# ttanv/funsearch-kubernetes-simulator

Hardware: AMD Instinct MI355X
Metric: policy evals/sec on 8,152-pod Alibaba trace at 1/2/4/8 GPUs; champion util/frag (higher is better)
Workload: dtype fp64; 1 GPU; model=composite_linear policy family, exact replay (reference-bit-identical scores), global_batch=49152, seq_len=8152, parallelism=islands: 4/GPU x 1 rank(s), single rank (no collectives), dist_backend=none, world_size=1, candidates_per_island=12288, backend=hip, heap_mode=auto, islands_async=True

## Files before the change

### csrc/hip/engine_host.hip.h

```cpp
#pragma once

#include <hip/hip_runtime.h>
#include <pybind11/numpy.h>
#include <rocprofiler-sdk-roctx/roctx.h>
#include <pybind11/pybind11.h>

#include <algorithm>
#include <cmath>
#include <cstdio>
#include <cstdlib>
#include <mutex>
#include <cstring>
#include <memory>
#include <string>
#include <vector>

namespace fks_host {

namespace py = pybind11;
using namespace fksd;

#define HIP_OK(expr)                                                                    \
  do {                                                                                  \
    hipError_t _e = (expr);                                                             \
// ... 704 lines not shown
      if (c5) {
        if (s.fam_spec != FAM_COMPOSITE_LINEAR || !g)
          throw std::invalid_argument("256-node profiling: composite batch with verified reciprocals and an HBM heap");
        HIP_OK(fksk::launch_c5_prof(P, lds, s.stream, a));
      } else {
        HIP_OK(fksk::launch_builtin_prof(g, P, lds, s.stream, a));
      }
    }
    finish(s);
    py::array_t<uint64_t> prof({(py::ssize_t)P, (py::ssize_t)8});
    HIP_OK(hipMemcpyAsync(prof.mutable_data(), s.prof.p, (size_t)P * 64, hipMemcpyDeviceToHost, s.stream));
    py::array_t<double> tab = wait(0);
    HIP_OK(hipStreamSynchronize(s.stream));
    return py::make_tuple(tab, prof);
  }

  py::tuple profile_rows(py::array_t<int32_t, py::array::c_style | py::array::forcecast> fam,
                         py::array_t<double, py::array::c_style | py::array::forcecast> weights) {
    if (!rows_ok_) throw std::invalid_argument("row kernel needs <= 16 nodes");
    HIP_OK(hipSetDevice(device_));
    Slot& s = idle_slot(0);
    stage_builtin(s, fam.data(), weights.data(), (int)fam.size());
    const int waves = launch_rows(s, true);
    finish(s);
    py::array_t<uint64_t> prof({(py::ssize_t)waves, (py::ssize_t)kRowProfWords});
    HIP_OK(hipMemcpyAsync(prof.mutable_data(), s.prof.p, (size_t)waves * 8 * kRowProfWords, hipMemcpyDeviceToHost,
                          s.stream));
    py::array_t<double> tab = wait(0);
    HIP_OK(hipStreamSynchronize(s.stream));
    return py::make_tuple(tab, prof);
  }

  py::dict info() const {
    py::dict d;
    d["device"] = device_; d["arch"] = arch_; d["num_cus"] = num_cus_;
    d["heap_bytes_per_policy"] = (int64_t)heap_bytes_;
    d["lds_heap_ok"] = lds_heap_ok_;
    d["npass"] = npass_;
    d["heap_mode"] = heap_mode_;
    d["n_slots"] = (int)slots_.size();
    d["heap_top_hbm"] = heap_top_for(0, false);
    d["row_kernel_ok"] = rows_ok_;
    d["row_kernel"] = row_mode_;
    d["row_heap_top"] = row_top();
    d["row_waves_per_cu"] = row_layout(FAM_COMPOSITE_LINEAR).second;
    d["row_wave_share"] = row_share_;
    d["fast_div"] = (int)W_.fast_div;
    d["cap_recips"] = W_.cap_recip[1] != 0.0;
    d["frag_recip"] = W_.z_tg != 0.0;
    d["row_composite_waves"] = comp_waves_;
    d["stack_bytes"] = (int64_t)stack_bytes_;
    d["row_flat"] = row_flat_;
    d["native_rows_last"] = last_native_rows_;
    d["native_waves_last"] = last_native_waves_;
    d["native_duo_top_last"] = last_duo_top_;
    d["native_duo_per_cu_last"] = last_duo_per_cu_;
    d["native_duo_reg_cap"] = fksk::native_duo_blocks_per_cu(0);
    d["native_inflight"] = native_inflight_;
    d["max_events"] = (int64_t)max_events_;
    d["wave_duo"] = wave_duo_;
    d["wave_duo_heap_top"] = npass_ >= 4 ? heap_top_for(0, false, true) : 0;
    size_t mfree = 0, mtotal = 0;
    if (hipMemGetInfo(&mfree, &mtotal) == hipSuccess) {
      d["mem_used_mb"] = (int64_t)((mtotal - mfree) >> 20);
      d["mem_total_mb"] = (int64_t)(mtotal >> 20);
    }
    return d;
  }

  bool would_use_hbm(int P) const { return use_gheap(P); }
  bool would_use_rows(int) const { return use_rows(); }
  int n_slots() const { return (int)slots_.size(); }

 private:
  static constexpr size_t kMaxLds = 160 * 1024;
  static constexpr int kWeightWords = kWeights;
  static constexpr size_t kSimds = 4;
  static constexpr size_t kPoliciesPerCu = kSimds * FKS_LIGHT_WAVES;
  static constexpr size_t kNp2PoliciesPerCu = kSimds * FKS_NP2_WAVES;
  static constexpr size_t kNp4PoliciesPerCu = kSimds * FKS_NP4_WAVES;
  static constexpr size_t kNp4DuoPoliciesPerCu = 2 * FKS_NP4_DUO_WAVES;
  static constexpr size_t kVmPoliciesPerCu = kSimds * FKS_VM_WAVES;

  void prepare_recips(py::dict d) {
    auto i32 = [&](const char* k) {
      return py::array_t<int32_t, py::array::c_style | py::array::forcecast>(d[k].cast<py::array>());
    };
    const auto ct = i32("cpu_total"), cl = i32("cpu_left"), mt = i32("mem_total"), ml = i32("mem_left"), ng = i32("ngpus");
    const auto pod = i32("pod");
    const int nn = (int)ct.size(), np = W_.n_pods;
    std::vector<std::pair<std::pair<int64_t, int64_t>, double>> cache;
    bool ok = true;
    std::vector<double> rec((size_t)nn * 3, 0.0), cm((size_t)std::max(np, 1), 0.0);
    std::vector<int32_t> per_class(256, 0);
    for (int r = 0; r < np; ++r) {
      const int32_t c = pod.data()[4 * r], m = pod.data()[4 * r + 1];
      ok = ok && c >= 0 && m >= 0;
      cm[r] = (double)c / (double)(m > 1 ? m : 1);
      const uint32_t pw = (uint32_t)pod.data()[4 * r + 3];
      if ((pw >> 16) & 0xFF) ++per_class[pw >> 24];
    }
    max_class_pods_ = *std::max_element(per_class.begin(), per_class.end());
    {
      const auto gl = i32("gpu_left"), gt = i32("gml_total"), gml = i32("gml_left");
      bool b = ok;
      for (int n = 0; n < nn && b; ++n) {
// ... 246 lines not shown
    if (profiled) HIP_OK(fksk::launch_builtin_rows_prof(kf, P, waves, s.queue.as<uint32_t>(), s.qbase, lds, s.stream, a));
    else HIP_OK(fksk::launch_builtin_rows(kf, P, waves, s.queue.as<uint32_t>(), s.qbase, lds, s.stream, a));
    s.qbase += (uint32_t)P + (uint32_t)waves * kRowsPerWave;
    return waves;
  }

  int duo_top(int want) const {
    const int entries = row_heap_entries(W_.n_pods);
    if (native_duo_top_ >= 0) {
      int T = 1;
      while (T < entries - 1 && 2 * T + 1 <= native_duo_top_) T = 2 * T + 1;
      return T;
    }
    const int reg_cap = std::max(1, fksk::native_duo_blocks_per_cu(0));
    const int need = std::min(reg_cap, std::max(1, (want + num_cus_ - 1) / std::max(1, num_cus_)));
    auto per_cu = [&](int T) {
      const size_t lds = duo_lds_bytes(W_.n_pods, T);
      if (lds > kMaxLds) return 0;
      return std::max(0, fksk::native_duo_blocks_per_cu(lds));
    };
    int T = 63;
    while (T < entries - 1 && per_cu(2 * T + 1) >= std::max(2, need)) T = 2 * T + 1;
    return T;
  }

  void launch_rows_native(Slot& s, int P, size_t fn_bytes, const int64_t* kc_dev, bool profiled = false) {
    const int ra = native_rows_opt_ > 0 ? native_rows_opt_ : (native_duo_ || P <= 2 * num_cus_ ? 1 : kRowsPerWave);
    DevWorkload Wl = W_;
    const int entries = row_heap_entries(W_.n_pods);
    if (ra == 1 && native_duo_) {
      const int T = duo_top(std::max(P, native_inflight_));
      Wl.heap_top = T;
      last_duo_top_ = T;
      last_duo_per_cu_ = fksk::native_duo_blocks_per_cu(duo_lds_bytes(W_.n_pods, T));
      const size_t lds = duo_lds_bytes(W_.n_pods, T);
      if (lds > kMaxLds) throw std::invalid_argument("native duo layout exceeds the 160 KiB LDS");
      s.gheap.reserve((size_t)entries * 8 * (size_t)P);
      if (profiled) s.prof.reserve((size_t)P * 128);
      const fksk::BuiltinArgs a{Wl, nullptr, nullptr, nullptr, nullptr, s.res.as<DevResult>(),
                                s.gheap.as<uint64_t>(), profiled ? s.prof.as<uint64_t>() : nullptr,
                                s.h_tab.dev<double>()};
      s.fused_table = true;
      const RowNativeArgs nat{s.h_in.dev<const uint64_t>(), kc_dev,
                              reinterpret_cast<const int32_t*>(s.h_in.dev<char>() + fn_bytes), nullptr, max_events_};
      if (std::getenv("FKS_DEBUG_LAUNCH"))
        std::fprintf(stderr, "[fks] native duo: P=%d T=%d lds=%zu per_cu=%d stream=%p\n", P, T, lds,
                     last_duo_per_cu_, (void*)s.stream);
      HIP_OK(fksk::launch_native_duo(P, lds, s.stream, a, nat));
      last_native_rows_ = 0;
      last_native_waves_ = 2 * P;
      return;
    }
    int T = 1;
    while (T < entries - 1 && rows_lds_bytes(W_.n_pods, 2 * T + 1, ra, true) <= kMaxLds / 2) T = 2 * T + 1;
    Wl.heap_top = T;
    const size_t lds = rows_lds_bytes(W_.n_pods, T, ra, true) + (profiled ? kRowProfBytes : 0);
    if (lds > kMaxLds) throw std::invalid_argument("native row kernel layout exceeds the 160 KiB LDS");
    const int per_cu = std::max(1, std::min(fksk::native_rows_waves_per_cu(lds), (int)(kMaxLds / ((lds + 2047) & ~size_t(2047)))));
    const int cap = std::max(1, (int)(row_share_ * per_cu * num_cus_));
    const int waves = std::max(1, std::min((P + ra - 1) / ra, cap));
    s.gheap.reserve((size_t)entries * 8 * (size_t)waves * kRowsPerWave);
    if (profiled) s.prof.reserve((size_t)waves * 8 * kRowProfWords);
    const fksk::BuiltinArgs a{Wl, nullptr, nullptr, nullptr, nullptr, s.res.as<DevResult>(),
                              s.gheap.as<uint64_t>(), profiled ? s.prof.as<uint64_t>() : nullptr, s.h_tab.dev<double>()};
    s.fused_table = true;
    const RowNativeArgs nat{s.h_in.dev<const uint64_t>(), kc_dev,
                            reinterpret_cast<const int32_t*>(s.h_in.dev<char>() + fn_bytes)};
    if (std::getenv("FKS_DEBUG_LAUNCH"))
      std::fprintf(stderr, "[fks] native rows: P=%d rows=%d waves=%d T=%d lds=%zu qbase=%u stream=%p\n", P, ra, waves, T,
                   lds, s.qbase, (void*)s.stream);
    HIP_OK(fksk::launch_native_rows(P, waves, ra, s.queue.as<uint32_t>(), s.qbase, lds, s.stream, a, nat));
    s.qbase += (uint32_t)P + (uint32_t)waves * (uint32_t)ra;
    last_native_rows_ = ra;
    last_native_waves_ = waves;
  }

  void launch_vm(Slot& s, int nregs) {
    const int P = s.P;
    const bool g = use_gheap(P);
    const DevWorkload Wl = launch_workload(g, nregs, true);
    const size_t lds = lds_bytes(g, Wl.heap_top, nregs);
    if (lds > kMaxLds) throw std::invalid_argument("heap + VM registers exceed the 160 KiB LDS");
    uint64_t* gh = g ? gheap_for(s, P) : nullptr;
    const fksk::VmArgs a{Wl, nullptr, table(s), s.res.as<DevResult>(), budget_, nregs, gh, nullptr};
    HIP_OK(fksk::launch_vm(npass_, g, P, lds, s.stream, a));
  }

  static void zero_queue(Slot& s) {
    static const uint64_t zeros[8] = {0, 0, 0, 0, 0, 0, 0, 0};
    HIP_OK(hipMemcpyAsync(s.queue.p, zeros, 64, hipMemcpyHostToDevice, s.stream));
    HIP_OK(hipStreamSynchronize(s.stream));
  }

  void finish(Slot& s) {
    const int P = s.P;
    if (!s.fused_table)
      hipLaunchKernelGGL(k_eval_reduce, dim3((P + 63) / 64), dim3(64), 0, s.stream, s.res.as<DevResult>(),
                         s.h_tab.dev<double>(), P);
    s.fused_table = false;
    HIP_OK(hipGetLastError());
    HIP_OK(hipEventRecord(s.done, s.stream));
    s.busy = true;
  }

  int device_ = 0;
  std::vector<std::unique_ptr<Slot>> slots_;
  DevWorkload W_;
  int npass_ = 1;
  size_t heap_bytes_ = 0, delmap_bytes_ = 0;
  bool lds_heap_ok_ = true;
  bool rows_ok_ = false;
  bool state_bounded_ = false;
  std::string row_mode_ = "auto";
  int row_top_opt_ = -1;
  double row_share_ = 1.0;
  bool native_duo_ = true;
  int native_rows_opt_ = 0;
  int native_inflight_ = 0;
  int native_duo_top_ = -1;
  int last_duo_top_ = 0, last_duo_per_cu_ = 0;
  int last_native_rows_ = 0, last_native_waves_ = 0;
  size_t row_min_lds_ = 0;
  int32_t max_class_pods_ = 0;
  int32_t max_gpu_milli_ = 0;
  static constexpr size_t kJitStackBytes = 2048;
  size_t stack_bytes_ = 0;
  bool row_flat_ = true;
  int comp_waves_ = 5;
  mutable std::vector<std::pair<int, int>> row_layout_cache_ = std::vector<std::pair<int, int>>(8, {0, 0});
  int num_cus_ = 0;
  std::string arch_;
  std::string heap_mode_ = "auto";
  int64_t budget_ = 0;
  uint32_t max_events_ = 0;
  int heap_top_opt_ = -1;
  bool partial_delmap_off_ = false;
  bool wave_duo_ = false;
  std::vector<void*> owned_;
};

}
```

### csrc/hip/replay_duo.hip.h

```cpp
#pragma once

#include "replay_rows.hip.h"

namespace fksd {

constexpr int kDuoRing = 64;
#ifndef FKS_DUO_SLEEP
#define FKS_DUO_SLEEP 1
#endif
constexpr uint32_t kDuoSpinCap = 1u << 26;
enum DuoReply : int32_t { DUO_NONE = 0, DUO_PLACED = 1, DUO_FAIL = 2, DUO_ABORT = 3 };

struct DuoBox {
  uint64_t ev[kDuoRing];
  uint64_t item;
  uint32_t head;
  uint32_t tail;
  uint32_t rseq;
  int32_t code;
  uint32_t term;
  uint32_t sabort;
  int32_t h_exc, n_repush, n_dropped;
};
constexpr int kDuoNodeInts = 16;
constexpr size_t kDuoSBytes = (size_t)kRow * kDuoNodeInts * 4 + (size_t)kRow * 32;
__host__ __device__ inline size_t duo_lds_bytes(int n_pods, int T) {
  return rows_lds_bytes(n_pods, T, 1, true) + ((sizeof(DuoBox) + 15) & ~size_t(15)) + kDuoSBytes;
}

__device__ __forceinline__ uint32_t duo_ld(FKS_LDS uint32_t* p) {
  return __hip_atomic_load(p, __ATOMIC_ACQUIRE, __HIP_MEMORY_SCOPE_WORKGROUP);
}
__device__ __forceinline__ void duo_st(FKS_LDS uint32_t* p, uint32_t v) {
  __hip_atomic_store(p, v, __ATOMIC_RELEASE, __HIP_MEMORY_SCOPE_WORKGROUP);
}


__device__ __forceinline__ void duo_reset(FKS_LDS DuoBox* box) {
  box->item = 0; box->head = 0; box->tail = 0; box->rseq = 0; box->code = DUO_NONE; box->term = 0;
  box->sabort = 0;
  box->h_exc = EXC_NONE; box->n_repush = 0; box->n_dropped = 0;
}

__device__ __forceinline__ bool duo_publish(FKS_LDS DuoBox* box, bool first, uint32_t k, uint32_t& tail_seen,
                                            uint64_t key, int32_t& hexc) {
  uint32_t spins = 0;
  while (k - tail_seen >= (uint32_t)kDuoRing) {
    tail_seen = duo_ld(&box->tail);
    if (k - tail_seen < (uint32_t)kDuoRing) break;
    if (duo_ld(&box->sabort)) return false;
    __builtin_amdgcn_s_sleep(FKS_DUO_SLEEP);
    if (++spins > kDuoSpinCap) { hexc = EXC_TIMEOUT; return false; }
  }
  if (first) box->ev[k % kDuoRing] = key;
  if (first) duo_st(&box->head, k + 1);
  return true;
}

__device__ __forceinline__ bool duo_verdict(FKS_LDS DuoBox* box, uint32_t k, int32_t& hexc) {
  uint32_t spins = 0;
  while (duo_ld(&box->rseq) != k + 1) {
    if (duo_ld(&box->sabort)) { hexc = EXC_TIMEOUT; return false; }
    __builtin_amdgcn_s_sleep(FKS_DUO_SLEEP);
    if (++spins > kDuoSpinCap) { hexc = EXC_TIMEOUT; return false; }
  }
  return true;
}

__device__ __forceinline__ void duo_term(FKS_LDS DuoBox* box, int32_t hexc, int n_repush, int n_dropped) {
  box->h_exc = hexc;
  box->n_repush = n_repush;
  box->n_dropped = n_dropped;
  duo_st(&box->term, 1u);
}

__device__ __forceinline__ bool duo_next(FKS_LDS DuoBox* box, uint32_t k, int32_t& exc) {
  uint32_t spins = 0;
  for (;;) {
    if (duo_ld(&box->head) > k) return true;
    if (duo_ld(&box->term)) return duo_ld(&box->head) > k;
// ... 69 lines not shown
    }
    pos = next;
    if (taken < 6) break;
  }
  if (target < 0) target = pos;
  if (j == 0) { hp.st(target, last); hp.mark(target, last); }
}

template <bool PROF = false>
__device__ void replay_duo(const DevWorkload& W, const DevWorkload* Wdev, uint64_t* gheap, DevResult* out,
                           RowNativeArgs nat, double* table, uint64_t* prof_out = nullptr, int slot = -1,
                           int hslot = -1) {
  uint64_t pacc[8] = {0, 0, 0, 0, 0, 0, 0, 0};
  uint64_t plast = 0;
  auto mark = [&](int ph) {
    if constexpr (PROF) {
      const uint64_t now = __builtin_amdgcn_s_memtime();
      pacc[ph] += now - plast;
      plast = now;
    }
  };
  auto flush = [&](int wv) {
    if constexpr (PROF) {
      if (lane_id() < 8) {
        uint64_t v = 0;
#pragma unroll
        for (int i = 0; i < 8; ++i) v = lane_id() == i ? pacc[i] : v;
        prof_out[16 * (size_t)blockIdx.x + 8 * wv + lane_id()] = v;
      }
    }
  };
  auto cold = [&]() {
    const DevWorkload* g = reinterpret_cast<const DevWorkload*>(uniu64(reinterpret_cast<uint64_t>(Wdev)));
    asm volatile("" : "+s"(g));
    return const_ptr(g);
  };
  extern __shared__ uint64_t lds_raw[];
  const int lane = lane_id();
  const int wave = (int)(threadIdx.x >> 6);
  const int p = slot >= 0 ? slot : (int)blockIdx.x;
  const int hs = hslot >= 0 ? hslot : p;
  const int N = W.n_pods;
  const int T = W.heap_top;
  const int lb = W.low_bits, nb = W.node_bits, rb = W.rank_bits;
  const int tshift = rb + lb;
  const uint64_t time_max = (W.time_bits >= 63) ? ~0ull : ((1ull << W.time_bits) - 1);
  int jv = lane & 15;
  const bool node_valid = jv < W.n_nodes;

  FKS_LDS uint64_t* lds = lds_ptr(lds_raw);
  FKS_LDS int32_t* cls_lds = reinterpret_cast<FKS_LDS int32_t*>(lds + kRowsPerWave * kWeights);
  FKS_LDS char* rowbase = reinterpret_cast<FKS_LDS char*>(lds + kRowsPerWave * kWeights) + kRowClassBytes;
  FKS_LDS int32_t* ntab = cls_lds + kRow * kRowClassSlots;
  FKS_LDS int64_t* kcp = reinterpret_cast<FKS_LDS int64_t*>(rowbase + rows_row_bytes(N, T));
  FKS_LDS DuoBox* box = reinterpret_cast<FKS_LDS DuoBox*>(reinterpret_cast<FKS_LDS char*>(lds) + rows_lds_bytes(N, T, 1, true));
  FKS_LDS int32_t* sstate = reinterpret_cast<FKS_LDS int32_t*>(reinterpret_cast<FKS_LDS char*>(box) +
                                                                ((sizeof(DuoBox) + 15) & ~size_t(15)));
  FKS_LDS uint64_t* sacc = reinterpret_cast<FKS_LDS uint64_t*>(sstate + kRow * kDuoNodeInts);

  if (wave == 0) {
    if (lane < W.n_classes) cls_lds[lane] = *global_ptr(&W.class_value[lane]);
    fill_node_tables(W, ntab, lane);
    if (lane == 0) {
      box->item = 0; box->head = 0; box->tail = 0; box->rseq = 0; box->code = DUO_NONE; box->term = 0;
      box->sabort = 0;
      box->h_exc = EXC_NONE; box->n_repush = 0; box->n_dropped = 0;
    }
  } else {
    const FKS_GLOBAL int64_t* ksrc = global_ptr(nat.kc + *global_ptr(&nat.koff[p]));
    for (int i = lane; i < kKcLds; i += kWave) kcp[i] = ksrc[i];
  }
  __syncthreads();
  if (wave == 1 && lane >= kRow) return;

  if (wave == 0) {
    RowHeap heap;
    heap.delmap = reinterpret_cast<FKS_LDS uint32_t*>(rowbase);
    heap.top = reinterpret_cast<FKS_LDS uint64_t*>(rowbase + (size_t)lds_delmap_words(N) * 4);
    heap.h = global_ptr(gheap + (size_t)hs * row_heap_entries(N));
    heap.bind();
    heap.T = T;
    heap.lb = lb;
    heap.j = jv;
    heap.rbase = 0;
    heap.anc = heap.dir = 0;
    uint64_t anc64 = 0, dir64 = 0;
    for (int x = lane; x > 0 && x < 63; x = (x - 1) >> 1) {
      const int a = (x - 1) >> 1;
      anc64 |= 1ull << a;
      if ((x & 1) == 0) dir64 |= 1ull << a;
    }
    const FKS_GLOBAL u64x2* heap_src = reinterpret_cast<const FKS_GLOBAL u64x2*>(global_ptr(W.heap0p));
    for (int i = lane; i < row_heap_entries(N) / 2; i += kWave) {
      const u64x2 v = heap_src[i];
      if (2 * i < T + 1) *reinterpret_cast<FKS_LDS u64x2*>(heap.top + 2 * i) = v;
      else *reinterpret_cast<FKS_GLOBAL u64x2*>(heap.h + 2 * i) = v;
    }
    for (int i = lane; i < lds_delmap_words(N); i += kWave) heap.delmap[i] = 0u;
    __builtin_amdgcn_s_waitcnt(0);
    int n = N, n_repush = 0, n_dropped = 0;
    int32_t hexc = EXC_NONE;
    uint32_t k = 0, tail_seen = 0;
    auto publish = [&](uint64_t key) -> bool {
      uint32_t spins = 0;
      while (k - tail_seen >= (uint32_t)kDuoRing) {
        tail_seen = duo_ld(&box->tail);
        if (k - tail_seen < (uint32_t)kDuoRing) break;
        if (duo_ld(&box->sabort)) return false;
// ... 386 lines not shown
```

### csrc/hip/replay_rows.hip.h

```cpp
#pragma once

#include "replay.hip.h"
#include "scorers.hip.h"
#include "jit_abi.h"

namespace fksd {

#ifndef FKS_ROW_FLAT
#define FKS_ROW_FLAT 1
#endif
constexpr int kFamNative = 100;
constexpr int kRowCompositeW5 = 5;
constexpr int kRowCompositeSplit = 6;
struct RowNativeArgs {
  const uint64_t* fn;
  const int64_t* kc;
  const int32_t* koff;
  const uint32_t* abort = nullptr;
  uint32_t max_events = 0;
};
struct ServiceCtl {
  uint32_t* claimed;
  const uint32_t* published;
  const uint32_t* stop;
  uint32_t* done;
  const uint32_t* qslot;
  uint32_t* started;
  uint32_t nq;
  uint32_t max_idle_polls;
  uint64_t* cost;
};

constexpr int kRow = 16;
constexpr int kRowsPerWave = 4;
constexpr int kRowClassSlots = 4;
constexpr int kRowMaxHeap = (1 << 17) - 2;

__host__ __device__ inline int row_heap_entries(int n_pods) { return (n_pods + 2 + 63) & ~63; }

__device__ __forceinline__ uint32_t row_ballot(bool p, int rbase) {
  return (uint32_t)(ballot(p) >> rbase) & 0xFFFFu;
}
template <int N>
__device__ __forceinline__ uint32_t row_ror32(uint32_t v) {
  return (uint32_t)__builtin_amdgcn_mov_dpp((int)v, 0x120 + N, 0xF, 0xF, false);
}
template <int N>
__device__ __forceinline__ uint64_t row_ror64(uint64_t v) {
  return ((uint64_t)row_ror32<N>((uint32_t)(v >> 32)) << 32) | row_ror32<N>((uint32_t)v);
}
__device__ __forceinline__ uint64_t row_max_u64(uint64_t v) {
  uint64_t o;
  o = row_ror64<8>(v); v = o > v ? o : v;
  o = row_ror64<4>(v); v = o > v ? o : v;
  o = row_ror64<2>(v); v = o > v ? o : v;
  o = row_ror64<1>(v); v = o > v ? o : v;
  return v;
}
__device__ __forceinline__ int64_t row_sum_i64(int64_t v) {
  uint64_t u = (uint64_t)v;
  u += row_ror64<8>(u);
  u += row_ror64<4>(u);
  u += row_ror64<2>(u);
  u += row_ror64<1>(u);
  return (int64_t)u;
}
__device__ __forceinline__ int row_read(int v, int rbase, int k) {
  return __builtin_amdgcn_ds_bpermute((rbase + k) << 2, v);
}

typedef uint64_t u64x2 __attribute__((ext_vector_type(2)));

template <bool FLAT = FKS_ROW_FLAT != 0>
struct RowHeapT {
  FKS_GLOBAL uint64_t* h;
  FKS_LDS uint64_t* top;
  int T;
  FKS_LDS uint32_t* delmap;
  int lb;
  int j, rbase;
  uint32_t anc, dir;

  uint64_t* gtop;
  uint64_t* gh;
  __device__ __forceinline__ void bind() {
    gtop = (uint64_t*)top;
    gh = (uint64_t*)h;
  }
  __device__ __forceinline__ uint64_t* slot(int i) const { return (i < T ? gtop : gh) + (i + 1); }
  __device__ __forceinline__ uint64_t ld(int i) const {
    if constexpr (FLAT) return *slot(i);
    else return i < T ? top[i + 1] : h[i + 1];
  }
  __device__ __forceinline__ void st(int i, uint64_t v) const {
    if constexpr (FLAT) {
      *slot(i) = v;
    } else {
      if (i < T) top[i + 1] = v;
      else h[i + 1] = v;
    }
  }
  __device__ __forceinline__ u64x2 ld_pair(int c) const {
    if constexpr (FLAT) return *reinterpret_cast<const u64x2*>(slot(c));
    if (c < T) return *reinterpret_cast<const FKS_LDS u64x2*>(top + c + 1);
    return *reinterpret_cast<const FKS_GLOBAL u64x2*>(h + c + 1);
  }
  __device__ __forceinline__ void mark(int pos, uint64_t v) const {
    const uint32_t bit = 1u << (pos & 31);
    const uint32_t data = (v & 3) == kDelKind ? bit : 0u;
    const uint32_t addr = (uint32_t)(uintptr_t)(delmap + (pos >> 5));
    asm volatile("ds_mskor_b32 %0, %1, %2" ::"v"(addr), "v"(bit), "v"(data) : "memory");
  }

  __device__ void pop_reinsert(int n, uint64_t last) const {
    const int k = j == 0 ? 0 : j < 3 ? 1 : j < 7 ? 2 : 3;
    const int ki = j - ((1 << k) - 1);
    constexpr int kRounds = 5;
    int pos = 0, target = -1;
#pragma unroll
    for (int rd = 0; rd < kRounds; ++rd) {
      if (2 * pos + 1 >= n) break;
      const int q = ((pos + 1) << k) - 1 + ki;
      const int c = 2 * q + 1;
      const bool valid = j < 15 && c < n;
      uint64_t vl = ~0ull, vr = ~0ull;
      if (valid) {
        const u64x2 pr = ld_pair(c);
        vl = pr.x;
        vr = pr.y;
      }
      const bool go_r = valid && (c + 1 < n) && !(vl < vr);
      const uint32_t m = row_ballot(go_r, rbase);
      const bool on = valid && ((m ^ dir) & anc) == 0;
      const uint32_t onm = row_ballot(on, rbase);
      const uint64_t v = go_r ? vr : vl;
      const uint32_t g = row_ballot(on && last < v, rbase);
      const int jl = g ? __ffs(g) - 1 : kRow;
      if (on && j < jl) {
        st(q, v);
        mark(q, v);
      }
      if (g) {
        target = row_read(q, rbase, jl);
        break;
      }
      const int jd = 31 - __clz(onm);
      const int nk = row_read(((c + (int)go_r) << 2) | k, rbase, jd);
      pos = nk >> 2;
      if ((nk & 3) < 3) break;
    }
    if (target < 0) target = pos;
    if (j == 0) { st(target, last); mark(target, last); }
  }

  __device__ void push(int n, uint64_t item) const {
    const int l = j + 1;
    const int anc = ((n + 1) >> l) - 1;
    const bool valid = n > 0 && anc >= 0;
    const uint64_t v = valid ? ld(anc) : 0;
    const bool gt = valid && item < v;
    const int J = __popc(row_ballot(gt, rbase));
    const int dst = ((n + 1) >> (l - 1)) - 1;
    if (gt) { st(dst, v); mark(dst, v); }
    const int aJ = J == 0 ? n : ((n + 1) >> J) - 1;
    if (j == 0) { st(aJ, item); mark(aJ, item); }
  }

  __device__ int first_deletion(int n) const {
    const int words = (n + 31) >> 5;
    for (int base = 0; base < words; base += kRow) {
      const int wi = base + j;
      uint32_t w = wi < words ? delmap[wi] : 0u;
      if (wi == words - 1 && (n & 31)) w &= (1u << (n & 31)) - 1;
      const uint32_t b = row_ballot(w != 0, rbase);
      if (b) {
        const int fl = __ffs(b) - 1;
        const uint32_t fw = (uint32_t)row_read((int)w, rbase, fl);
        return ((base + fl) << 5) + (__ffs(fw) - 1);
      }
    }
    return -1;
  }
};
using RowHeap = RowHeapT<>;

struct RowAcc {
  uint64_t lo, hi;
  int32_t count;
  int32_t inexact;
  __device__ void init() { lo = hi = 0; count = 0; inexact = 0; }
  __device__ void add(int k, double v, int j) {
    const bool mine = j == k;
    const uint64_t bits = (uint64_t)__double_as_longlong(v);
    if (mine) ++count;
    if (bits == 0) return;
    const int E = (int)(bits >> 52);
    const uint64_t M = (bits & ((1ull << 52) - 1)) | (1ull << 52);
    const int shift = E - 979;
    bool bad = E == 0 || E >= 0x7FF || shift > 126 - 53;
    uint64_t tl, th;
    if (shift >= 0) {
      tl = shift < 64 ? M << shift : 0ull;
      th = shift == 0 ? 0ull : shift < 64 ? M >> (64 - shift) : M << (shift - 64);
    } else {
      bad = bad || shift <= -53 || (M & ((1ull << (-shift)) - 1)) != 0;
      tl = M >> (-shift & 63);
      th = 0;
    }
    if (bad) {
      if (mine) inexact |= 1;
      return;
    }
    if (mine) {
      lo += tl;
      hi += th + (lo < tl);
      if (hi >> 62) inexact |= 1;
    }
  }
  __device__ void add_unit(int k, double v, int j) {
    const bool mine = j == k;
    const uint64_t bits = (uint64_t)__double_as_longlong(v);
    if (mine) ++count;
    if (bits == 0) return;
    const int s = (int)(bits >> 52) - 979;
    const uint64_t M = (bits & ((1ull << 52) - 1)) | (1ull << 52);
    const uint64_t tl = M << (s & 63), th = M >> ((64 - s) & 63);
    if (mine) {
      if (s < 13 || s > 44) inexact |= 1;
      lo += tl;
      hi += th + (lo < tl);
    }
// ... 28 lines not shown
constexpr int kNodeRecips = 6;
constexpr int kCapRecips = 10;
constexpr int kRowClassBytes =
    (kRow * kRowClassSlots * 4 + kRow * kNodeConsts * 4 + kRow * kNodeRecips * 8 + kCapRecips * 8 + 15) & ~15;
__device__ __forceinline__ FKS_LDS double* row_node_recips(FKS_LDS int32_t* ntab) {
  return reinterpret_cast<FKS_LDS double*>(ntab + kRow * kNodeConsts);
}
__device__ __forceinline__ FKS_LDS double* row_cap_recips(FKS_LDS int32_t* ntab) {
  return row_node_recips(ntab) + kRow * kNodeRecips;
}
__device__ __forceinline__ int32_t row_sum_i32(int32_t v) {
  v += (int32_t)row_ror32<8>((uint32_t)v);
  v += (int32_t)row_ror32<4>((uint32_t)v);
  v += (int32_t)row_ror32<2>((uint32_t)v);
  v += (int32_t)row_ror32<1>((uint32_t)v);
  return v;
}
__device__ __forceinline__ uint32_t row_min_u32(uint32_t v) {
  v = min(v, row_ror32<8>(v));
  v = min(v, row_ror32<4>(v));
  v = min(v, row_ror32<2>(v));
  v = min(v, row_ror32<1>(v));
  return v;
}
__device__ __forceinline__ double max_nn(double a, double b) {
  double r;
  asm("v_max_f64 %0, %1, %2" : "=v"(r) : "v"(a), "v"(b));
  return r;
}
__device__ __forceinline__ double row_max_f64(double v) {
  v = max_nn(v, __longlong_as_double((long long)row_ror64<8>((uint64_t)__double_as_longlong(v))));
  v = max_nn(v, __longlong_as_double((long long)row_ror64<4>((uint64_t)__double_as_longlong(v))));
  v = max_nn(v, __longlong_as_double((long long)row_ror64<2>((uint64_t)__double_as_longlong(v))));
  v = max_nn(v, __longlong_as_double((long long)row_ror64<1>((uint64_t)__double_as_longlong(v))));
  return v;
}
__device__ __forceinline__ void fill_node_tables(const DevWorkload& W, FKS_LDS int32_t* ntab, int lane) {
  if (lane < kRow) {
    ntab[lane * kNodeConsts + 0] = W.cpu_total[lane];
    ntab[lane * kNodeConsts + 1] = W.mem_total[lane];
    ntab[lane * kNodeConsts + 2] = W.ngpus[lane];
    ntab[lane * kNodeConsts + 3] = W.gml_total[lane * kGmax];
    FKS_LDS double* z = row_node_recips(ntab);
#pragma unroll
    for (int k = 0; k < 3; ++k) z[lane * kNodeRecips + k] = W.node_recip[lane * 3 + k];
    const int32_t ct = W.cpu_total[lane], mt = W.mem_total[lane], ng = W.ngpus[lane];
    z[lane * kNodeRecips + 3] = (double)(ct > 1 ? ct : 1);
    z[lane * kNodeRecips + 4] = (double)(mt > 1 ? mt : 1);
    z[lane * kNodeRecips + 5] = (double)(ng > 1 ? ng : 1);
  }
  if (lane <= kGmax) row_cap_recips(ntab)[lane] = W.cap_recip[lane];
}
constexpr int kRowColdBytes = 32;
__host__ __device__ inline size_t rows_row_bytes(int n_pods, int T) {
  return (size_t)lds_delmap_words(n_pods) * 4 + (size_t)(T + 1) * 8 + kRowColdBytes;
}
__host__ __device__ inline size_t rows_lds_bytes(int n_pods, int T, int rows = kRowsPerWave, bool kc = false) {
  return (size_t)kRowsPerWave * kWeights * 8 + kRowClassBytes + (size_t)rows * rows_row_bytes(n_pods, T) +
         (kc ? (size_t)rows * kKcLds * 8 : 0);
}

struct RowNoProf {
  __device__ void start(FKS_LDS uint64_t*) {}
  __device__ void mark(int) {}
  __device__ void kinds(int) {}
  __device__ void flush(uint64_t*) {}
};
struct RowProf {
  FKS_LDS uint64_t* c;
  __device__ void start(FKS_LDS uint64_t* at) {
    c = at;
    if (lane_id() < 16) c[lane_id()] = lane_id() == 8 ? __builtin_amdgcn_s_memtime() : 0;
  }
  __device__ void mark(int ph) {
    const uint64_t now = __builtin_amdgcn_s_memtime();
    if (lane_id() == __builtin_amdgcn_readfirstlane(lane_id())) {
      c[ph] += now - c[8];
      c[8] = now;
    }
  }
  __device__ void kinds(int cat) {
    const int m = (ballot(cat == 1) != 0 ? 1 : 0) | (ballot(cat == 2) != 0 ? 2 : 0) | (ballot(cat == 3) != 0 ? 4 : 0);
    if (m != 0 && lane_id() == __builtin_amdgcn_readfirstlane(lane_id())) c[8 + m] += 1;
  }
  __device__ void flush(uint64_t* o) {
    if (lane_id() < 16) o[lane_id()] = lane_id() == 8 ? 0 : c[lane_id()];
  }
};
constexpr int kRowProfBytes = 128;
constexpr int kRowProfWords = 16;

__device__ __forceinline__ void write_row_result(const RowAcc& acc, int jv, int rbase, int32_t processed, int32_t exc,
                                                 int64_t n_repush, int n_dropped, uint64_t hsh, DevResult* o,
                                                 double* table_row) {
  const int64_t n_snap = row_read(acc.count, rbase, 0);
  const int64_t n_frag = row_read(acc.count, rbase, 4);
  const int inexact = row_ballot(jv < 5 && (acc.inexact & 1) != 0, rbase) != 0;
  if (jv < 5) {
    o->acc_lo[jv] = acc.lo;
    o->acc_hi[jv] = acc.hi;
  }
  if (jv == 0) {
    o->n_events = processed;
    o->n_snap = n_snap;
    o->n_frag = n_frag;
    o->n_unplaced = n_dropped;
    o->n_repush = n_repush;
    o->max_nodes = 0;
    o->hash = hsh;
    o->exc = exc;
    o->inexact = inexact;
// ... 13 lines not shown
      const double overall = (avg[0] + avg[1] + avg[2] + avg[3]) / 4.0;
      const double pen = avg[4] < 0.1 ? avg[4] : 0.1;
      double sc = overall - pen;
      sc = sc < 1.0 ? sc : 1.0;
      score = sc > 0.0 ? sc : 0.0;
    }
    const bool ok = exc == EXC_NONE;
    double v = 0.0;
    switch (jv) {
      case 0: v = score; break;
      case 1: case 2: case 3: case 4: case 5: v = avg[jv - 1]; break;
      case 6: v = (double)n_snap; break;
      case 7: v = (double)n_frag; break;
      case 8: v = (double)processed; break;
      case 9: v = (double)n_dropped; break;
      case 10: v = (double)exc; break;
      case 11: v = (double)inexact; break;
      case 12: v = (double)(hsh >> 11); break;
      default: break;
    }
    if (!ok && jv != 10) v = 0.0;
    if (jv < 13) table_row[jv] = v;
  }
}

template <int FAM, class Prof = RowNoProf, bool FLAT = FKS_ROW_FLAT != 0>
__device__ void replay_rows(const DevWorkload& W, const DevWorkload* Wdev, const int32_t* fam, const double* weights,
                            uint64_t* gheap, DevResult* out, int P, uint32_t* queue, uint32_t qbase,
                            uint64_t* prof_out = nullptr, RowNativeArgs nat = RowNativeArgs{nullptr, nullptr, nullptr},
                            int rows_active = kRowsPerWave, double* table = nullptr) {
  constexpr bool kNative = FAM == kFamNative;
  const int ra = kNative ? rows_active : kRowsPerWave;
  extern __shared__ uint64_t lds_raw[];
  const int lane = lane_id();
  const int row = lane >> 4;
  const int rbase = lane & 48;
  const int slot = blockIdx.x * kRowsPerWave + row;
  const int N = W.n_pods;
  const int T = W.heap_top;
  const int lb = W.low_bits, nb = W.node_bits, rb = W.rank_bits;
  const int tshift = rb + lb;
  const uint64_t time_max = (W.time_bits >= 63) ? ~0ull : ((1ull << W.time_bits) - 1);
  int jv = lane & 15;
  const bool node_valid = jv < W.n_nodes;

  FKS_LDS uint64_t* lds = lds_ptr(lds_raw);
  FKS_LDS double* wl = reinterpret_cast<FKS_LDS double*>(lds) + row * kWeights;
  FKS_LDS int32_t* cls_lds = reinterpret_cast<FKS_LDS int32_t*>(lds + kRowsPerWave * kWeights);
  FKS_LDS char* rowbase = reinterpret_cast<FKS_LDS char*>(lds + kRowsPerWave * kWeights) + kRowClassBytes +
                          (size_t)row * rows_row_bytes(N, T);
  if (lane < W.n_classes) cls_lds[lane] = *global_ptr(&W.class_value[lane]);
  FKS_LDS int32_t* ntab = cls_lds + kRow * kRowClassSlots;
  fill_node_tables(W, ntab, lane);
  RowHeapT<FLAT> heap;
  heap.delmap = reinterpret_cast<FKS_LDS uint32_t*>(rowbase);
  heap.top = reinterpret_cast<FKS_LDS uint64_t*>(rowbase + (size_t)lds_delmap_words(N) * 4);
  heap.h = global_ptr(gheap + (size_t)slot * row_heap_entries(N));
  heap.bind();
  heap.T = T;
  heap.lb = lb;
  heap.j = jv;
  heap.rbase = rbase;
  heap.anc = heap.dir = 0;
  for (int x = jv; x > 0 && x < 15; x = (x - 1) >> 1) {
    const int a = (x - 1) >> 1;
    heap.anc |= 1u << a;
    if ((x & 1) == 0) heap.dir |= 1u << a;
  }
  const FKS_GLOBAL u64x2* heap_src = reinterpret_cast<const FKS_GLOBAL u64x2*>(global_ptr(W.heap0p));

  auto claim = [&]() {
    if (kNative && row >= ra) return P;
    const int c = jv == 0 ? (int)(__hip_atomic_fetch_add(queue, 1u, __ATOMIC_RELAXED, __HIP_MEMORY_SCOPE_AGENT) - qbase) : 0;
    return row_read(c, rbase, 0);
  };
  int p = claim();
  int family = FAM;
  NodeRegs<1, !kNative> nr;
  auto load_consts = [&]() {
    const FKS_LDS int32_t* e = ntab + jv * kNodeConsts;
    nr.cpu_total[0] = e[0];
    nr.mem_total[0] = e[1];
    nr.ngpus[0] = e[2];
    nr.gmt1[0] = e[3];
  };
  uint32_t wcp[kRowClassSlots / 2];
  auto wcount = [&](int sl) -> uint32_t { return (wcp[sl >> 1] >> (16 * (sl & 1))) & 0xFFFFu; };
  RowAcc acc;
  int32_t processed = 0, next_fire = INT32_MAX;
  int n = 0;
  FKS_LDS uint64_t* rcs = heap.top + (T + 1);
  FKS_LDS uint32_t* rcn = reinterpret_cast<FKS_LDS uint32_t*>(rcs + 2);
  auto bump = [&](int k) {
    if (jv == 0) __hip_atomic_fetch_add(&rcn[k], 1u, __ATOMIC_RELAXED, __HIP_MEMORY_SCOPE_WORKGROUP);
  };
  int32_t exc = EXC_NONE;
  ProgFn prog = nullptr;
  bool feas_pro = false;
  FKS_LDS int64_t* kcp = reinterpret_cast<FKS_LDS int64_t*>(
      reinterpret_cast<FKS_LDS char*>(lds + kRowsPerWave * kWeights) + kRowClassBytes +
      (size_t)ra * rows_row_bytes(N, T)) + (size_t)row * kKcLds;

  auto begin = [&]() {
    if constexpr (kNative) {
      const uint64_t fne = *global_ptr(&nat.fn[p]);
      prog = prog_of(fne);
      feas_pro = prog_feas(fne);
      const FKS_GLOBAL int64_t* ksrc = global_ptr(nat.kc + *global_ptr(&nat.koff[p]));
      for (int i = jv; i < kKcLds; i += kRow) kcp[i] = ksrc[i];
    } else {
      wl[jv] = *global_ptr(&weights[(size_t)p * kWeights + jv]);
      if (FAM < 0) family = *global_ptr(&fam[p]);
    }
    const int words = row_heap_entries(N) / 2;
    for (int i = jv; i < words; i += kRow) {
      const u64x2 v = heap_src[i];
      if constexpr (FLAT) {
        *reinterpret_cast<u64x2*>((2 * i < T + 1 ? heap.gtop : heap.gh) + 2 * i) = v;
      } else {
        if (2 * i < T + 1) *reinterpret_cast<FKS_LDS u64x2*>(heap.top + 2 * i) = v;
        else *reinterpret_cast<FKS_GLOBAL u64x2*>(heap.h + 2 * i) = v;
      }
    }
    for (int i = jv; i < lds_delmap_words(N); i += kRow) heap.delmap[i] = 0u;
    const FKS_CONST DevWorkload* Wb = cold_ptr(Wdev);
    nr.cpu_left[0] = Wb->cpu_left0[jv];
    nr.mem_left[0] = Wb->mem_left0[jv];
    nr.gpu_left[0] = Wb->gpu_left0[jv];
#pragma unroll
    for (int g = 0; g < kGmax; ++g) {
      nr.g_init(0, g, Wb->gml_left0[jv * kGmax + g]);
    }
#pragma unroll
    for (int k = 0; k < kRowClassSlots / 2; ++k) wcp[k] = 0u;
    acc.init();
    processed = 0;
    rcn[0] = 0u; rcn[1] = 0u; rcn[2] = 0u;
    const double thr = Wb->thr_after_fire;
    rcs[1] = (uint64_t)__double_as_longlong(thr);
    if (Wb->n_fire > 0) {
      next_fire = (int32_t)*global_ptr(&Wb->snap_fire[0]);
    } else {
      int32_t c = 1;
      while ((double)c / (double)N < thr) ++c;
      next_fire = c;
    }
    rcs[0] = 0xcbf29ce484222325ull;
    exc = EXC_NONE;
    n = N;
    __builtin_amdgcn_s_waitcnt(0);
  };

  Prof prof;
  prof.start(reinterpret_cast<FKS_LDS uint64_t*>(reinterpret_cast<FKS_LDS char*>(lds) + rows_lds_bytes(N, T, ra, kNative)));
  bool have = p < P;
  if (have) begin();
  prof.mark(PH_EVAL);

  while (have) {
    asm volatile("" : "+v"(jv));
    heap.j = jv;
    int ecat = 0;
    do {
      const uint64_t top = heap.ld(0);
      const int rank = (int)((top >> lb) & ((1ull << rb) - 1));
      typedef int v4i __attribute__((ext_vector_type(4)));
      const v4i precv = *reinterpret_cast<const FKS_GLOBAL v4i*>(global_ptr(&W.pod[rank]));
      const uint64_t last = heap.ld(n - 1);
      --n;
      if (n > 0) heap.pop_reinsert(n, last);
      const int kind = (int)(top & 3);
      const int64_t t = (int64_t)(top >> tshift);
      PodView pod;
      pod.cpu = precv.x; pod.mem = precv.y; pod.dur = precv.z;
      pod.gmilli = precv.w & 0xFFFF; pod.ngpu = (precv.w >> 16) & 0xFF; pod.cls = (precv.w >> 24) & 0xFF;
      pod.ctime = t; pod.rank = rank;
      prof.mark(PH_POP);
// ... 34 lines not shown
          } else {
            s = BuiltinScorerDev<FAM>::template score_weights<1>(family, wq, 0, nr, pod, lexc);
          }
          if (lexc != EXC_NONE) { s = 0; sd = 0.0; }
        }
        const uint32_t bad = row_ballot(lexc != EXC_NONE, rbase);
        if (bad) {
          exc = row_read(lexc, rbase, __ffs(bad) - 1);
          break;
        }
        int best_node;
        if constexpr (kComp) {
          const double md = row_max_f64(sd);
          best_node = md > 0.0 ? __ffs(row_ballot(sd == md, rbase)) - 1 : -1;
        } else {
          const int64_t m = (int64_t)row_max_u64((uint64_t)s);
          best_node = m > 0 ? __ffs(row_ballot(s == m, rbase)) - 1 : -1;
        }
        uint64_t push_item = 0;
        prof.mark(PH_SCORE);

        if (best_node < 0) {
          const bool waits_new = kind == kFresh && pod.ngpu > 0;
          if (waits_new) {
#pragma unroll
            for (int sl = 0; sl < kRowClassSlots; ++sl)
              if (sl == (pod.cls >> 4) && jv == (pod.cls & 15)) wcp[sl >> 1] += 1u << (16 * (sl & 1));
          }
          if (waits_new || !acc.stash_valid()) {
            double frag = 0.0;
            uint32_t nzs = 0;
#pragma unroll
            for (int sl = kRowClassSlots - 1; sl >= 0; --sl) nzs = wcount(sl) > 0 ? (uint32_t)sl : nzs;
            bool any = false;
#pragma unroll
            for (int k = 0; k < kRowClassSlots / 2; ++k) any = any || wcp[k] != 0u;
            const int mcls = (int)row_min_u32(any ? nzs * kRow + (uint32_t)jv : 64u);
            if (mcls < 64) {
              const int mv = cls_lds[mcls];
              int32_t stranded = 0;
#pragma unroll
              for (int g = 0; g < kGmax; ++g) {
                const int l = nr.g(0, g);
                if (0 < l && l < mv) stranded += l;
              }
              stranded = row_sum_i32(node_valid ? stranded : 0);
              const int64_t tg = cold_ptr(Wdev)->tot_gmilli;
              frag = tg <= 0 ? 0.0 : W.z_tg != 0.0 ? div_by_recip((double)stranded, W.tot_gmilli_d, W.z_tg)
                                                   : (double)stranded / W.tot_gmilli_d;
            }
            acc.stash_unit(frag, jv);
          }
          acc.add_stash(jv);
          const int f = heap.first_deletion(n);
          if (f >= 0) {
            const uint64_t nt = (heap.ld(f) >> tshift) + 1;
            if (nt > time_max) { exc = EXC_UNSUPPORTED; break; }
            push_item = (nt << tshift) | ((uint64_t)rank << lb) | kRetry;
            bump(0);
          } else {
            bump(1);
          }
          if (cold_ptr(Wdev)->trace_hash) rcs[0] = mix_event(rcs[0], ((uint64_t)(uint32_t)rank << 2) | 2, (uint64_t)t);
          ecat = 3;
          prof.mark(PH_FAIL);
        } else {
          int gmask = 0, ok = 1;
          if (pod.ngpu > 0) {
            int myok = 1;
            const int mymask = pick_gpus<1>(nr, 0, pod.gmilli, pod.ngpu, cold_ptr(Wdev)->first_fit_alloc != 0, myok);
            const int packed = row_read(mymask | (myok << 8), rbase, best_node);
            gmask = packed & 0xFF;
            ok = packed >> 8;
          }
          if (!ok) { exc = EXC_ALLOC; break; }
          acc.stash_drop();
          if (jv == best_node) {
            nr.cpu_left[0] -= pod.cpu;
            nr.mem_left[0] -= pod.mem;
            nr.gpu_left[0] -= pod.ngpu;
#pragma unroll
            for (int g = 0; g < kGmax; ++g)
              if ((gmask >> g) & 1) nr.g_add(0, g, -pod.gmilli);
          }
          if (kind == kRetry && pod.ngpu > 0) {
#pragma unroll
            for (int sl = 0; sl < kRowClassSlots; ++sl)
              if (sl == (pod.cls >> 4) && jv == (pod.cls & 15)) wcp[sl >> 1] -= 1u << (16 * (sl & 1));
          }
          const uint64_t dt = (uint64_t)(t + pod.dur);
          if (t + pod.dur < 0 || dt > time_max) { exc = EXC_UNSUPPORTED; break; }
          push_item = (dt << tshift) | ((uint64_t)rank << lb) | ((uint64_t)gmask << (2 + nb)) |
                      ((uint64_t)best_node << 2) | kDelete;
          if (cold_ptr(Wdev)->trace_hash)
            rcs[0] = mix_event(rcs[0], ((uint64_t)(uint32_t)rank << 2), ((uint64_t)t << 8) ^ (uint64_t)best_node);
          ecat = 2;
          prof.mark(PH_COMMIT);
        }
        if (push_item != 0) {
          heap.push(n, push_item);
          ++n;
        }
      }

      ++processed;
      if (processed >= next_fire) {
        const FKS_CONST DevWorkload* Ws = cold_ptr(Wdev);
        int32_t gl_sum = 0;
#pragma unroll
// ... 42 lines not shown
```

Before: 106,000 policy_evals/s.

## Drop LDS deletion bitmap in row kernel; scan heap keys for first deletion

Measured after the change: 116,000 policy_evals/s, median of 6. 9.5% higher.

```diff
diff --git a/csrc/hip/engine_host.hip.h b/csrc/hip/engine_host.hip.h
--- a/csrc/hip/engine_host.hip.h
+++ b/csrc/hip/engine_host.hip.h
@@ -780,6 +780,7 @@
     d["stack_bytes"] = (int64_t)stack_bytes_;
     d["row_flat"] = row_flat_;
     d["native_rows_last"] = last_native_rows_;
+    d["native_rows_top_last"] = last_native_top_;
     d["native_waves_last"] = last_native_waves_;
     d["native_duo_top_last"] = last_duo_top_;
     d["native_duo_per_cu_last"] = last_duo_per_cu_;
@@ -1132,7 +1133,10 @@
       return;
     }
     int T = 1;
-    while (T < entries - 1 && rows_lds_bytes(W_.n_pods, 2 * T + 1, ra, true) <= kMaxLds / 2) T = 2 * T + 1;
+    while (T < entries - 1 && rows_lds_bytes(W_.n_pods, 2 * T + 1, ra, true) <= kMaxLds / 2 &&
+           (row_top_opt_ <= 0 || 2 * T + 1 <= row_top_opt_))
+      T = 2 * T + 1;
+    last_native_top_ = T;
     Wl.heap_top = T;
     const size_t lds = rows_lds_bytes(W_.n_pods, T, ra, true) + (profiled ? kRowProfBytes : 0);
     if (lds > kMaxLds) throw std::invalid_argument("native row kernel layout exceeds the 160 KiB LDS");
@@ -1199,7 +1203,7 @@
   int native_inflight_ = 0;
   int native_duo_top_ = -1;
   int last_duo_top_ = 0, last_duo_per_cu_ = 0;
-  int last_native_rows_ = 0, last_native_waves_ = 0;
+  int last_native_rows_ = 0, last_native_waves_ = 0, last_native_top_ = 0;
   size_t row_min_lds_ = 0;
   int32_t max_class_pods_ = 0;
   int32_t max_gpu_milli_ = 0;
diff --git a/csrc/hip/replay_duo.hip.h b/csrc/hip/replay_duo.hip.h
--- a/csrc/hip/replay_duo.hip.h
+++ b/csrc/hip/replay_duo.hip.h
@@ -25,7 +25,7 @@
 constexpr int kDuoNodeInts = 16;
 constexpr size_t kDuoSBytes = (size_t)kRow * kDuoNodeInts * 4 + (size_t)kRow * 32;
 __host__ __device__ inline size_t duo_lds_bytes(int n_pods, int T) {
-  return rows_lds_bytes(n_pods, T, 1, true) + ((sizeof(DuoBox) + 15) & ~size_t(15)) + kDuoSBytes;
+  return rows_lds_bytes(n_pods, T, 1, true, true) + ((sizeof(DuoBox) + 15) & ~size_t(15)) + kDuoSBytes;
 }
 
 __device__ __forceinline__ uint32_t duo_ld(FKS_LDS uint32_t* p) {
@@ -201,8 +201,8 @@
   FKS_LDS int32_t* cls_lds = reinterpret_cast<FKS_LDS int32_t*>(lds + kRowsPerWave * kWeights);
   FKS_LDS char* rowbase = reinterpret_cast<FKS_LDS char*>(lds + kRowsPerWave * kWeights) + kRowClassBytes;
   FKS_LDS int32_t* ntab = cls_lds + kRow * kRowClassSlots;
-  FKS_LDS int64_t* kcp = reinterpret_cast<FKS_LDS int64_t*>(rowbase + rows_row_bytes(N, T));
-  FKS_LDS DuoBox* box = reinterpret_cast<FKS_LDS DuoBox*>(reinterpret_cast<FKS_LDS char*>(lds) + rows_lds_bytes(N, T, 1, true));
+  FKS_LDS int64_t* kcp = reinterpret_cast<FKS_LDS int64_t*>(rowbase + rows_row_bytes(N, T, true));
+  FKS_LDS DuoBox* box = reinterpret_cast<FKS_LDS DuoBox*>(reinterpret_cast<FKS_LDS char*>(lds) + rows_lds_bytes(N, T, 1, true, true));
   FKS_LDS int32_t* sstate = reinterpret_cast<FKS_LDS int32_t*>(reinterpret_cast<FKS_LDS char*>(box) +
                                                                 ((sizeof(DuoBox) + 15) & ~size_t(15)));
   FKS_LDS uint64_t* sacc = reinterpret_cast<FKS_LDS uint64_t*>(sstate + kRow * kDuoNodeInts);
diff --git a/csrc/hip/replay_rows.hip.h b/csrc/hip/replay_rows.hip.h
--- a/csrc/hip/replay_rows.hip.h
+++ b/csrc/hip/replay_rows.hip.h
@@ -71,7 +71,7 @@
 
 typedef uint64_t u64x2 __attribute__((ext_vector_type(2)));
 
-template <bool FLAT = FKS_ROW_FLAT != 0>
+template <bool FLAT = FKS_ROW_FLAT != 0, bool MAP = true>
 struct RowHeapT {
   FKS_GLOBAL uint64_t* h;
   FKS_LDS uint64_t* top;
@@ -106,6 +106,7 @@
     return *reinterpret_cast<const FKS_GLOBAL u64x2*>(h + c + 1);
   }
   __device__ __forceinline__ void mark(int pos, uint64_t v) const {
+    if constexpr (!MAP) return;
     const uint32_t bit = 1u << (pos & 31);
     const uint32_t data = (v & 3) == kDelKind ? bit : 0u;
     const uint32_t addr = (uint32_t)(uintptr_t)(delmap + (pos >> 5));
@@ -167,6 +168,7 @@
   }
 
   __device__ int first_deletion(int n) const {
+    static_assert(MAP, "bitmap-free heaps scan the keys: scan_deletion");
     const int words = (n + 31) >> 5;
     for (int base = 0; base < words; base += kRow) {
       const int wi = base + j;
@@ -177,6 +179,26 @@
         const int fl = __ffs(b) - 1;
         const uint32_t fw = (uint32_t)row_read((int)w, rbase, fl);
         return ((base + fl) << 5) + (__ffs(fw) - 1);
+      }
+    }
+    return -1;
+  }
+
+  __device__ int scan_deletion(int n, uint64_t& key) const {
+    const int lim = n + 2 * j;
+    for (int c = 2 * j - 1; c < lim; c += 2 * kRow) {
+      u64x2 pr = {0, 0};
+      if (c < n) pr = ld_pair(c);
+      const bool d0 = c >= 0 && c < n && ((uint32_t)pr.x & 3u) == (uint32_t)kDelKind;
+      const bool d1 = c + 1 < n && ((uint32_t)pr.y & 3u) == (uint32_t)kDelKind;
+      const uint32_t b0 = row_ballot(d0, rbase);
+      const uint32_t b = b0 | row_ballot(d1, rbase);
+      if (b) {
+        const int fl = __ffs(b) - 1;
+        const uint64_t mine = d0 ? pr.x : pr.y;
+        key = ((uint64_t)(uint32_t)row_read((int)(mine >> 32), rbase, fl) << 32) |
+              (uint32_t)row_read((int)(uint32_t)mine, rbase, fl);
+        return c - 2 * j + 1 + 2 * fl - (int)((b0 >> fl) & 1u);
       }
     }
     return -1;
@@ -311,11 +333,12 @@
   if (lane <= kGmax) row_cap_recips(ntab)[lane] = W.cap_recip[lane];
 }
 constexpr int kRowColdBytes = 32;
-__host__ __device__ inline size_t rows_row_bytes(int n_pods, int T) {
-  return (size_t)lds_delmap_words(n_pods) * 4 + (size_t)(T + 1) * 8 + kRowColdBytes;
-}
-__host__ __device__ inline size_t rows_lds_bytes(int n_pods, int T, int rows = kRowsPerWave, bool kc = false) {
-  return (size_t)kRowsPerWave * kWeights * 8 + kRowClassBytes + (size_t)rows * rows_row_bytes(n_pods, T) +
+__host__ __device__ inline size_t rows_row_bytes(int n_pods, int T, bool map = false) {
+  return (map ? (size_t)lds_delmap_words(n_pods) * 4 : 0) + (size_t)(T + 1) * 8 + kRowColdBytes;
+}
+__host__ __device__ inline size_t rows_lds_bytes(int n_pods, int T, int rows = kRowsPerWave, bool kc = false,
+                                                 bool map = false) {
+  return (size_t)kRowsPerWave * kWeights * 8 + kRowClassBytes + (size_t)rows * rows_row_bytes(n_pods, T, map) +
          (kc ? (size_t)rows * kKcLds * 8 : 0);
 }
 
@@ -435,9 +458,8 @@
   if (lane < W.n_classes) cls_lds[lane] = *global_ptr(&W.class_value[lane]);
   FKS_LDS int32_t* ntab = cls_lds + kRow * kRowClassSlots;
   fill_node_tables(W, ntab, lane);
-  RowHeapT<FLAT> heap;
-  heap.delmap = reinterpret_cast<FKS_LDS uint32_t*>(rowbase);
-  heap.top = reinterpret_cast<FKS_LDS uint64_t*>(rowbase + (size_t)lds_delmap_words(N) * 4);
+  RowHeapT<FLAT, false> heap;
+  heap.top = reinterpret_cast<FKS_LDS uint64_t*>(rowbase);
   heap.h = global_ptr(gheap + (size_t)slot * row_heap_entries(N));
   heap.bind();
   heap.T = T;
@@ -505,7 +527,6 @@
         else *reinterpret_cast<FKS_GLOBAL u64x2*>(heap.h + 2 * i) = v;
       }
     }
-    for (int i = jv; i < lds_delmap_words(N); i += kRow) heap.delmap[i] = 0u;
     const FKS_CONST DevWorkload* Wb = cold_ptr(Wdev);
     nr.cpu_left[0] = Wb->cpu_left0[jv];
     nr.mem_left[0] = Wb->mem_left0[jv];
@@ -646,9 +667,10 @@
             acc.stash_unit(frag, jv);
           }
           acc.add_stash(jv);
-          const int f = heap.first_deletion(n);
+          uint64_t anchor = 0;
+          const int f = heap.scan_deletion(n, anchor);
           if (f >= 0) {
-            const uint64_t nt = (heap.ld(f) >> tshift) + 1;
+            const uint64_t nt = (anchor >> tshift) + 1;
             if (nt > time_max) { exc = EXC_UNSUPPORTED; break; }
             push_item = (nt << tshift) | ((uint64_t)rank << lb) | kRetry;
             bump(0);
```
